# HKUST-Aerial-Robotics/Omni-swarm

Measured on AMD Instinct MI355X. Metric: keyframes/sec (4x fisheye 600x480) + p50 loop-match ms @ 100k-frame DB, higher is better.
Workload: dtype f16

## Files before the change

### omni-swarm_amd/csrc/config.hip

```cpp
#include "config.h"

#include <atomic>
#include <cerrno>
#include <climits>
#include <cstdlib>

namespace omni {

const CfgOption kCfgOptions[CFG_COUNT] = {
    {"OMNI_CONV_V1", 0, 0, 3, CFG_VARIANT, "fp16 3x3 layers: 0 = production (conv1a fused into the ping-pong conv1b, register-stationary cin=128); 1 = generic kernel, 2 = persistent LDS-DMA kernel, "
                                           "3 = ping-pong without the conv1a fusion -- 1-3 exist only in the test build of the library (lib_test/)"},
    {"OMNI_RS_TRN", -1, -1, 1, CFG_VARIANT, "register-stationary kernel of the unpooled cin=128 fp16 layers: tile orientation, -1 = the one with fewer tiles, 0 = plain, 1 = transposed"},
    {"OMNI_DET16", 1, 0, 1, CFG_VARIANT, "detector head of the fp16 and OMNI_PREC_SPLIT paths on v_mfma_f32_32x32x16_f16 with split (hi, lo) operands (0: the exact-f32 MFMA kernel)"},
    {"OMNI_SP_SPARSE_DESC", 1, 0, 1, CFG_VARIANT, "convDb + descriptor norm only at the cells around the key points (0: dense descriptor map)"},
    {"OMNI_SP_SPARSE_DA", 1, 0, 1, CFG_VARIANT, "convDa only at those cells too (fp16 and OMNI_PREC_SPLIT; 0: dense convDa)"},
    {"OMNI_SP_FUSED_CAND", 1, 0, 1, CFG_VARIANT, "getKeyPoints' threshold inside the detector head's epilogue + window masks from the candidate list (0: sp_cand_kernel re-reads the heat map)"},
    {"OMNI_SP_SPLIT_DB", 1, 0, 1, CFG_VARIANT, "OMNI_PREC_SPLIT: convDb + descriptor norm at the key points' cells with split (hi, lo) operands on the fp16 matrix cores (0: exact-f32 MFMA convolution)"},
    {"OMNI_SP_MASK_SKIP", 1, 0, 1, CFG_VARIANT, "fp16: the tiles inside the constant region of the fisheye mask are left out of the tile walk (0: every tile)"},
    {"OMNI_SP_MASK_SKIP_SPLIT", 1, 0, 1, CFG_VARIANT, "the same for OMNI_PREC_SPLIT"},
    {"OMNI_SPLIT_FUSE1A", 1, 0, 1, CFG_VARIANT, "OMNI_PREC_SPLIT: conv1a built inside the conv1b kernel from the u8 image (0: separate exact-f32 conv1a pass)"},
    {"OMNI_SPLIT_WINO", 7, 0, 15, CFG_VARIANT, "OMNI_PREC_SPLIT: the cin = 64 layers as Winograd F(2x2,3x3) kernels with split operands (conv_wino.hip), bit 0 = conv1b (with the conv1a "
                                                "fusion), 1 = conv2a, 2 = conv2b, 3 = conv3a (off by default: same time as the direct kernel, profiles/r06g); 0: the direct kernels of conv_split.hip"},
    {"OMNI_SPLIT_TRN", -1, -1, 1, CFG_VARIANT, "OMNI_PREC_SPLIT cin=128 kernel: tile orientation, as OMNI_RS_TRN"},
    {"OMNI_CONV_XCD", 1, 0, 1, CFG_VARIANT, "persistent convolution kernels derive (cout group, tile walk) from an XCD-aware block id: the cout groups of a pixel tile and its neighbours "
                                           "share one L2 (0: plain blockIdx; process-wide, same results either way)"},
    {"OMNI_SP_PROFILE_MASK", 0, 0, 1, CFG_TUNING, "omni_sp_profile times the stages with the fisheye mask on (what the key-frame pipeline runs)"},
    {"OMNI_PP_U8", 1, 0, 1, CFG_VARIANT, "fp16 conv1a inside conv1b's kernel: matrix-core operands straight from the image bytes (0: through the 256-entry u8 -> (hi, lo) table in LDS)"},
    {"OMNI_PP_TRACE", 0, 0, 1, CFG_DEBUG, "s_memtime trace of the ping-pong conv kernel on stderr"},
    {"OMNI_PP_DBG", 0, 0, 255, CFG_DEBUG, "ping-pong conv kernel timing ablations (WRONG results)"},
    {"OMNI_RS_TRACE", 0, 0, 1, CFG_DEBUG, "s_memtime trace of the register-stationary kernel"},
    {"OMNI_SPLIT_TRACE", 0, 0, 1, CFG_DEBUG, "s_memtime trace of the split-precision kernel"},
    {"OMNI_SPLIT_DBG", 0, 0, 3, CFG_DEBUG, "split-precision kernel timing ablations: 1 = no stores, 2 = every DMA reads tile 0 (WRONG results)"},
    {"OMNI_WINO_TRACE", 0, 0, 1, CFG_DEBUG, "s_memtime trace of the Winograd split kernel"},
    {"OMNI_ROCTX", 0, 0, 1, CFG_DEBUG, "roctx ranges around upload / SuperPoint / MobileNetVLAD / post-processing / BF match / index add + search / exchange and the host loop's "
                                      "stages (rocprofv3 --marker-trace; the library is resolved by dlopen)"},
    {"OMNI_VLAD_BIG", 0, 0, 128, CFG_TUNING, "64 / 128: the 64- / 128-pixel tiles of the unfused block kernel (measured slower at 600x480)"},
    {"OMNI_VLAD_STEM_FUSE", 1, 0, 1, CFG_VARIANT, "stem + block 0 in one kernel (0: two kernels)"},
    {"OMNI_VLAD_UNFUSED", 0, 0, 1, CFG_VARIANT, "1: every block as expand / depthwise / project launches"},
    {"OMNI_VLAD_MFMA", 1, 0, 1, CFG_VARIANT, "late blocks' 1x1 convolutions on the matrix cores"},
    {"OMNI_VLAD_SBLOCK", 1, 0, 1, CFG_VARIANT, "fused split-fp16 block kernel (vlad_s.hip)"},
    {"OMNI_VLAD_MBLOCK_PX", 2048, 0, 1 << 24, CFG_TUNING, "fused matrix-core block kernel for blocks of at most this many input pixels per image (0 disables)"},
    {"OMNI_VLAD_MFMA_PX", 0, 0, 1 << 24, CFG_TUNING, "> 0: matrix-core 1x1 convolutions for blocks of at most this many input pixels per image (default 2048)"},
    {"OMNI_VLAD_FC_MFMA", 1, 0, 1, CFG_VARIANT, "the final FC on the matrix cores (0: VALU kernel)"},
    {"OMNI_VLAD_MBLOCK_CPW", 0, 0, 64, CFG_TUNING, "hidden-layer split of the matrix-core block kernel: chunks per workgroup (0 = no split; measured: does not pay)"},
    {"OMNI_VLAD_SB_LDSPAD", 0, 0, 160 * 1024, CFG_DEBUG, "extra LDS bytes per workgroup of the split block kernel (occupancy A/B)"},
// ... 119 lines not shown
```

### omni-swarm_amd/csrc/conv.h

```cpp
#pragma once
#include "common.h"
#include "tile_walk.h"

namespace omni {

#define CONV_TH 8
#define CONV_TW 32
#define RS_TH 6
#define RS_TW 32
int conv_rs_pool_tile_rows();
#define CONV_COUT_TILE 64
#define CONV_CIN_CHUNK 64

static inline size_t conv_packed_elems(int cin, int cout, int ksize) { return (size_t)cin * cout * ksize * ksize; }

void conv_pack_weights_f16(const float* w_oihw, int cin, int cout, int ksize, __half* out);
void conv_pack_weights_f32(const float* w_oihw, int cin, int cout, int ksize, float* out);

struct ConvArgs {
    const void* in;
    void* out;
    const void* w_packed;
    const float* bias;
    int batch, H, W, cin, cout, ksize;
    int in_cstride = 0;
    bool relu, pool;
    bool out_f32;
    int n_cu = 0;
    const void* zero_page = nullptr;
    float split_inv = 0.f;
    int variant = 0;
    int skip_ty0 = 0, skip_ty1 = 0, skip_tx0 = 0, skip_tx1 = 0;
};
int conv_mfma(hipStream_t stream, int precision, const ConvArgs& a);
int conv_read_pixel_f16(hipStream_t stream, const void* map, int Ho, int Wo, int C, int y, int x, void* vec);
int conv_fill_rect_f16(hipStream_t stream, void* map, int batch, int Ho, int Wo, int C, int y0, int y1, int x0, int x1, const void* vec);
int conv_read_pixel_bytes(hipStream_t stream, const void* map, int64_t row_bytes, int64_t org_bytes, int pix_bytes, int y, int x, void* vec);
int conv_fill_rect_bytes(hipStream_t stream, void* map, int batch, int64_t img_bytes, int64_t row_bytes, int64_t org_bytes, int pix_bytes, int y0, int y1, int x0, int x1,
                         const void* vec);

float conv_pack_weights_split(const float* w_oihw, int cin, int cout, uint16_t* out);
float conv_split_act_scale();
int conv_split(hipStream_t stream, const ConvArgs& a);
int conv1a_split(hipStream_t stream, const uint8_t* gray, int stride, int batch, int H, int W, int fisheye_mask, const float* w, const float* bias,
                 const float* u8_lut, void* out_split, int skip_tr0 = 0, int skip_tr1 = 0);
int split_to_nchw_f32(hipStream_t stream, const void* in_split, float* out, int batch, int C, int H, int W);
void conv1a_split_pack_fused(const float* w , const float* bias , uint16_t* frag );
int conv1ab_split_fused(hipStream_t stream, const ConvArgs& a, const uint8_t* gray, int gstride, int fisheye_mask, const void* w1a_frag, const uint32_t* lut_hl);
float conv_pack_weights_wino(const float* w_oihw, int cin, int cout, uint16_t* out);
// ... 59 lines not shown
```

### omni-swarm_amd/csrc/conv.hip

```cpp
#include "config.h"
#include "conv.h"
#include <type_traits>

namespace omni {

typedef _Float16 half8_t __attribute__((ext_vector_type(8)));
typedef _Float16 half4_t __attribute__((ext_vector_type(4)));
typedef float floatx16 __attribute__((ext_vector_type(16)));
typedef float floatx4 __attribute__((ext_vector_type(4)));

template <typename T, int KG, int EPL>
static void pack_weights(const float* w, int cin, int cout, int ks, T* out) {
    const int taps = ks * ks, n_ct = cout / 64, n_ch = cin / 64;
    size_t o = 0;
    for (int ct = 0; ct < n_ct; ++ct)
        for (int ch = 0; ch < n_ch; ++ch)
            for (int tap = 0; tap < taps; ++tap)
                for (int kg = 0; kg < KG; ++kg)
                    for (int m = 0; m < 2; ++m)
                        for (int l = 0; l < 64; ++l)
                            for (int e = 0; e < EPL; ++e) {
                                const int co = ct * 64 + m * 32 + (l & 31);
                                const int ci = ch * 64 + kg * (64 / KG) + (l >> 5) * EPL + e;
                                const float v = w[((size_t)co * cin + ci) * taps + tap];
// ... 810 lines not shown
static int launch_conv_pp(hipStream_t st, const ConvArgs& a, int n_cu) {
    static const int dbg = config_process()[CFG_PP_DBG];
    switch (dbg >> 2) {
        case 1: return launch_conv_pp_abl<POOL, 1>(st, a, n_cu, dbg & 3);
        case 2: return launch_conv_pp_abl<POOL, 2>(st, a, n_cu, dbg & 3);
        case 3: return launch_conv_pp_abl<POOL, 3>(st, a, n_cu, dbg & 3);
        default: return launch_conv_pp_abl<POOL, 0>(st, a, n_cu, dbg & 3);
    }
}

template <int J, int N, typename F>
__device__ __forceinline__ void spl2_for_each(F&& f) {
    if constexpr (J < N) { f(std::integral_constant<int, J>{}); spl2_for_each<J + 1, N>(f); }
}
#define CSP_KP 8
#define RS_ITH (RS_TH + 2)
#define RS_ITW (RS_TW + 2)
#define RS_PIX (RS_ITH * RS_ITW)
#define RS_CHUNKS (RS_PIX * 16)
#define RS_BUF_BYTES (RS_PIX * 256)
#define RS_SMEM (2 * RS_BUF_BYTES + 512)

template <int L>
__device__ __forceinline__ void rs_read(uint32_t row_base , int n, int hh, half8_t& dst) {
    constexpr int kx = L / 64, r = (L / 8) % 8, kg = L % 8;
    constexpr int pc = r * RS_ITW + kx;
    const uint32_t addr = (row_base + pc * 256 + ((((pc + n) & 15) ^ hh) << 4)) ^ (kg << 5);
    asm volatile("ds_read_b128 %0, %1" : "=v"(dst) : "v"(addr));
}
template <int N>
__device__ __forceinline__ void rs_wait(half8_t& f) { asm volatile("s_waitcnt lgkmcnt(%1)" : "+v"(f) : "i"(N)); }

template <int L, typename IssueFn>
__device__ __forceinline__ void rs_steps(uint32_t row_base, int n, int hh, const half8_t (&wreg)[72], floatx16 (&acc)[RS_TH], half8_t (&fb)[3],
                                         IssueFn& issue_piece) {
    if constexpr (L < 192) {
        constexpr int kx = L / 64, r = (L / 8) % 8, kg = L % 8;
        if constexpr (L + 2 < 192) rs_read<L + 2>(row_base, n, hh, fb[(L + 2) % 3]);
        rs_wait<(L + 2 < 192) ? 2 : (L + 1 < 192 ? 1 : 0)>(fb[L % 3]);
        __builtin_amdgcn_sched_barrier(0);
        if constexpr (r >= 0 && r < RS_TH) acc[r] = __builtin_amdgcn_mfma_f32_32x32x16_f16(wreg[(0 * 3 + kx) * 8 + kg], fb[L % 3], acc[r], 0, 0, 0);
        if constexpr (r - 1 >= 0 && r - 1 < RS_TH) acc[r - 1] = __builtin_amdgcn_mfma_f32_32x32x16_f16(wreg[(1 * 3 + kx) * 8 + kg], fb[L % 3], acc[r - 1], 0, 0, 0);
        if constexpr (r - 2 >= 0 && r - 2 < RS_TH) acc[r - 2] = __builtin_amdgcn_mfma_f32_32x32x16_f16(wreg[(2 * 3 + kx) * 8 + kg], fb[L % 3], acc[r - 2], 0, 0, 0);
        __builtin_amdgcn_sched_barrier(0);
        rs_steps<L + 1>(row_base, n, hh, wreg, acc, fb, issue_piece);
    }
}

__global__ void __launch_bounds__(256, 1)
conv3x3_c128_rs_kernel(const _Float16* __restrict__ in, _Float16* __restrict__ out, const _Float16* __restrict__ wp,
                       const float* __restrict__ bias, int H, int W, int cout, int n_cg, int tiles_x, int tiles_y, int batch, int relu,
                       const char* __restrict__ zero_page ,
                       unsigned long long* trace ,
                       TileWalk wk ) {
    extern __shared__ __attribute__((aligned(16))) char smem_raw[];
    const uint32_t lds0 = (uint32_t)(uintptr_t)(__attribute__((address_space(3))) char*)smem_raw;
    const int tid = threadIdx.x, lane = tid & 63;
    const int wave = __builtin_amdgcn_readfirstlane(tid >> 6);
    const int n = lane & 31, hh = lane >> 5;
    const bool tr = trace != nullptr && blockIdx.x == 0 && tid == 0;
    int tk = 0;
    const int bid = xcd_block_id(wk.xcd);
    const int cg = bid % n_cg, wg = bid / n_cg, nwg = gridDim.x / n_cg;
    const int tiles_per_img = wk.act;
    const int total = batch * tiles_per_img;
    const int g32 = cg * 4 + wave;

    half8_t wreg[72];
    {
        const _Float16* wbase = wp + (int64_t)(g32 >> 1) * 2 * 9 * 4096 + (g32 & 1) * 512 + lane * 8;
#pragma unroll
        for (int s2 = 0; s2 < 72; ++s2) {
            const int tap = s2 >> 3, ch = (s2 >> 2) & 1, kg4 = s2 & 3;
            wreg[s2] = *reinterpret_cast<const half8_t*>(wbase + ((ch * 9 + tap) * 4 + kg4) * 1024);
        }
    }
    float* const bias_lds = reinterpret_cast<float*>(smem_raw + 2 * RS_BUF_BYTES);
    if (tid < 128) bias_lds[tid] = bias[cg * 128 + tid];

    auto tile_origin = [&](int t, int& b, int& ty0, int& tx0) {
        b = t / tiles_per_img;
        int ry, rx;
        tile_walk_rc<false>(wk, tiles_x, t - b * tiles_per_img, ry, rx);
        ty0 = ry * RS_TH; tx0 = rx * RS_TW;
    };
    uint32_t goff[17];
    uint32_t hx[4] = {0, 0, 0, 0};
#pragma unroll
    for (int j = 0; j < 17; ++j) {
        const int idx = (wave * 17 + j) * 64 + lane;
        const int pix = idx >> 4, phys = idx & 15;
        const int iy = pix / RS_ITW, ix = pix - iy * RS_ITW;
        goff[j] = (uint32_t)((iy * W + ix) * 256 + ((phys ^ (pix & 15)) << 4));
        hx[j / 5] |= (uint32_t)ix << (6 * (j % 5));
    }
    const uint32_t in_img_bytes = (uint32_t)H * W * 256u;
    auto issue = [&](int t, int which) {
        int b, ty0, tx0;
        tile_origin(t, b, ty0, tx0);
        const int y0 = ty0 - 1, x0 = tx0 - 1;
        const auto rsrc = __builtin_amdgcn_make_buffer_rsrc(const_cast<_Float16*>(in) + (int64_t)b * H * W * 128, 0, in_img_bytes, 0x00020000);
        const uint32_t sorg = (uint32_t)((y0 * W + x0) * 256);
        char* base = smem_raw + which * RS_BUF_BYTES + wave * 17 * 1024;
#pragma unroll
        for (int j = 0; j < 17; ++j) {
            const uint32_t x = (uint32_t)(x0 + (int)((hx[j / 5] >> (6 * (j % 5))) & 63u));
            const uint32_t voff = x < (uint32_t)W ? goff[j] + sorg : 0x80000000u;
#if __HIP_DEVICE_COMPILE__
            __builtin_amdgcn_raw_ptr_buffer_load_lds(rsrc, (__attribute__((address_space(3))) void*)(base + j * 1024), 16, voff, 0, 0, 0);
#else
            (void)rsrc; (void)base; (void)voff;
#endif
        }
    };
    int t = wg;
    if (t < total) issue(t, 0);
    asm volatile("s_waitcnt vmcnt(0)" ::: "memory");
    __syncthreads();

    int cur = 0;
    for (; t < total; t += nwg, cur ^= 1) {
        const int tn = t + nwg;
        if (tr && tk < 8) { trace[tk * 8 + 0] = __builtin_amdgcn_s_memtime(); trace[tk * 8 + 6] = (unsigned long long)t; }
        if (tn < total) issue(tn, cur ^ 1);
        if (tr && tk < 8) trace[tk * 8 + 1] = __builtin_amdgcn_s_memtime();
        auto issue_piece = [&](int) {};
        const uint32_t row_base = lds0 + cur * RS_BUF_BYTES + n * 256;
        floatx16 acc[RS_TH];
#pragma unroll
        for (int f = 0; f < RS_TH; ++f)
#pragma unroll
            for (int i = 0; i < 16; ++i) acc[f][i] = 0.f;
        half8_t fb[3];
        rs_read<0>(row_base, n, hh, fb[0]);
        rs_read<1>(row_base, n, hh, fb[1]);
        __builtin_amdgcn_sched_barrier(0);
        rs_steps<0>(row_base, n, hh, wreg, acc, fb, issue_piece);
        if (tr && tk < 8) trace[tk * 8 + 2] = __builtin_amdgcn_s_memtime();

        {
            int b, ty0, tx0;
            tile_origin(t, b, ty0, tx0);
            const int ox = tx0 + n;
            float4 bs[4];
#pragma unroll
            for (int g = 0; g < 4; ++g) bs[g] = *reinterpret_cast<const float4*>(bias_lds + wave * 32 + 8 * g + 4 * hh);
#pragma unroll
            for (int f2 = 0; f2 < RS_TH / 2; ++f2) {
                const int oy = ty0 + 2 * f2;
                float v[16];
#pragma unroll
                for (int i = 0; i < 16; ++i) {
                    const float q = vmax_med3(acc[2 * f2][i], acc[2 * f2 + 1][i]);
                    v[i] = vmax_med3(q, dpp_swap_pairs(q));
                }
                _Float16* o = out + (((int64_t)b * (H >> 1) + (oy >> 1)) * (W >> 1) + (ox >> 1)) * cout + g32 * 32;
                store_frag16<false>(v, bs, o, hh, relu, (oy < H) && (ox < W) && !(n & 1));
            }
        }
        if (tr && tk < 8) trace[tk * 8 + 3] = __builtin_amdgcn_s_memtime();
        asm volatile("s_waitcnt vmcnt(0)" ::: "memory");
        if (tr && tk < 8) trace[tk * 8 + 4] = __builtin_amdgcn_s_memtime();
        __syncthreads();
        if (tr && tk < 8) { trace[tk * 8 + 5] = __builtin_amdgcn_s_memtime(); ++tk; }
    }
}

static int launch_conv_rs(hipStream_t st, const ConvArgs& a, int n_cu) {
    auto kfn = conv3x3_c128_rs_kernel;
    OMNI_HIP_TRY(hipFuncSetAttribute((const void*)kfn, hipFuncAttributeMaxDynamicSharedMemorySize, (int)RS_SMEM));
    const int tiles_x = cdiv(a.W, RS_TW), tiles_y = cdiv(a.H, RS_TH), n_cg = a.cout / 128;
    TileWalk wk;
    if (int rc = tile_walk_plan(wk, "conv_rs", tiles_x, tiles_y, a.skip_ty0, a.skip_ty1, a.skip_tx0, a.skip_tx1)) return rc;
    wk.xcd = config_process()[CFG_CONV_XCD];
    const int total = a.batch * wk.act;
    const int per_cg = tile_walk_grid(n_cu, n_cg, total);
    OMNI_REQUIRE(a.zero_page, OMNI_ERR_INVALID, "conv: ConvArgs.zero_page is not set");
    const char* zero_page = reinterpret_cast<const char*>(a.zero_page);
    static const bool want_trace = config_process()[CFG_RS_TRACE] != 0;
    static unsigned long long* trace_dev = nullptr;
    if (want_trace) {
        if (!trace_dev) OMNI_HIP_TRY(hipMalloc((void**)&trace_dev, 64 * 8));
        OMNI_HIP_TRY(hipMemsetAsync(trace_dev, 0, 64 * 8, st));
    }
    hipLaunchKernelGGL(kfn, dim3(per_cg * n_cg), dim3(256), RS_SMEM, st, reinterpret_cast<const _Float16*>(a.in),
                       reinterpret_cast<_Float16*>(a.out), reinterpret_cast<const _Float16*>(a.w_packed), a.bias, a.H, a.W, a.cout, n_cg,
                       tiles_x, tiles_y, a.batch, a.relu ? 1 : 0, zero_page, want_trace ? trace_dev : nullptr, wk);
    OMNI_LAUNCH_CHECK();
    if (want_trace) {
        unsigned long long h[64];
        OMNI_HIP_TRY(hipMemcpyAsync(h, trace_dev, sizeof(h), hipMemcpyDeviceToHost, st));
        OMNI_HIP_TRY(hipStreamSynchronize(st));
        static int launches = 0;
        if (launches++ / 4 == 5)
            for (int k = 0; k < 8; ++k)
                fprintf(stderr, "rs trace H=%d W=%d cout=%d tile %llu (ty %llu tx %llu): issue %llu mfma %llu epilogue %llu wait %llu zerofix+barrier %llu | total %llu\n",
                        a.H, a.W, a.cout, h[k * 8 + 6], (h[k * 8 + 6] % (tiles_x * tiles_y)) / tiles_x, (h[k * 8 + 6] % (tiles_x * tiles_y)) % tiles_x,
                        h[k * 8 + 1] - h[k * 8], h[k * 8 + 2] - h[k * 8 + 1], h[k * 8 + 3] - h[k * 8 + 2], h[k * 8 + 4] - h[k * 8 + 3],
                        h[k * 8 + 5] - h[k * 8 + 4], h[k * 8 + 5] - h[k * 8]);
    }
    return OMNI_OK;
}

#define RS2_RING 3
template <int TH> struct Rs2Cfg {
    static constexpr int ITH = TH + 2, PIX = ITH * RS_ITW, NPIECES = (PIX * 16 + 63) / 64, PPW = (NPIECES + 3) / 4, BUF = NPIECES * 1024, NL = 3 * ITH * 8;
    static constexpr size_t smem() { return 2 * (size_t)BUF + 512; }
};
template <int L, int ITH>
__device__ __forceinline__ void rs2_read(uint32_t row_base , int n, int hh, half8_t& dst) {
    constexpr int kx = L / (ITH * 8), r = (L / 8) % ITH, kg = L % 8;
    constexpr int pc = r * RS_ITW + kx;
    const uint32_t addr = (row_base + pc * 256 + ((((pc + n) & 15) ^ hh) << 4)) ^ (kg << 5);
    asm volatile("ds_read_b128 %0, %1" : "=v"(dst) : "v"(addr));
}
template <int TH> constexpr int rs2_nmfma(int L) { const int r = (L / 8) % (TH + 2); int c = 0; for (int ky = 0; ky < 3; ++ky) if (r - ky >= 0 && r - ky < TH) ++c; return c; }
template <int TH> constexpr int rs2_count_before(int L, int want) { int c = 0; for (int l = 0; l < L; ++l) c += rs2_nmfma<TH>(l) == want ? 1 : 0; return c; }
// ... 206 lines not shown
    static DynSmemState smem_state;
    OMNI_HIP_TRY(ensure_dyn_smem(smem_state, (const void*)kfn, Rs2Cfg<TH>::smem()));
    const int tiles_x = cdiv(a.W, TRN ? TH : RS_TW), tiles_y = cdiv(a.H, TRN ? RS_TW : TH), n_cg = a.cout / 128;
    OMNI_REQUIRE((int64_t)a.H * a.W * 256 < (1ll << 31) && (int64_t)a.H * a.W * a.cout * 2 < (1ll << 31), OMNI_ERR_INVALID, "conv_rs2: image too large for 32-bit offsets");
    TileWalk wk;
    if (int rc = TRN ? tile_walk_plan(wk, "conv_rs2", tiles_x, tiles_y, 0, 0, 0, 0)
                     : tile_walk_plan(wk, "conv_rs2", tiles_x, tiles_y, a.skip_ty0, a.skip_ty1, a.skip_tx0, a.skip_tx1)) return rc;
    wk.xcd = config_process()[CFG_CONV_XCD];
    const int total = a.batch * wk.act;
    const int per_cg = tile_walk_grid(n_cu, n_cg, total);
    hipLaunchKernelGGL(kfn, dim3(per_cg * n_cg), dim3(256), Rs2Cfg<TH>::smem(), st, reinterpret_cast<const _Float16*>(a.in), reinterpret_cast<_Float16*>(a.out),
                       reinterpret_cast<const _Float16*>(a.w_packed), a.bias, a.H, a.W, a.cout, n_cg, tiles_x, tiles_y, a.batch, a.relu ? 1 : 0, wk);
    OMNI_LAUNCH_CHECK();
    return OMNI_OK;
}
int conv_rs_pool_tile_rows() { return RS_TH; }

template <int S, bool TRN>
__device__ __forceinline__ void spc_steps(uint32_t base, const half8_t (&wreg)[72], floatx16& acc, half8_t (&fb)[3]) {
    if constexpr (S < 72) {
        constexpr int o = S / 8, kg = S % 8, tap = TRN ? o : (o % 3) * 3 + o / 3;
        if constexpr (S + 2 < 72) {
            constexpr int o2 = (S + 2) / 8, kg2 = (S + 2) % 8, tap2 = TRN ? o2 : (o2 % 3) * 3 + o2 / 3;
            asm volatile("ds_read_b128 %0, %1 offset:%2" : "=v"(fb[(S + 2) % 3]) : "v"(base), "i"(tap2 * 256 + kg2 * 32));
        }
        asm volatile("s_waitcnt lgkmcnt(%1)" : "+v"(fb[S % 3]) : "i"((S + 2 < 72) ? 2 : (S + 1 < 72 ? 1 : 0)));
        __builtin_amdgcn_sched_barrier(0);
        acc = __builtin_amdgcn_mfma_f32_32x32x16_f16(wreg[tap * 8 + kg], fb[S % 3], acc, 0, 0, 0);
        __builtin_amdgcn_sched_barrier(0);
        spc_steps<S + 1, TRN>(base, wreg, acc, fb);
    }
// ... 221 lines not shown
int conv_mfma(hipStream_t st, int precision, const ConvArgs& a) {
    OMNI_REQUIRE(a.cin % 64 == 0 && a.cout % 64 == 0, OMNI_ERR_INVALID, "conv_mfma: cin=%d cout=%d must be multiples of 64", a.cin, a.cout);
    OMNI_REQUIRE(a.ksize == 1 || a.ksize == 3, OMNI_ERR_INVALID, "conv_mfma: ksize=%d", a.ksize);
    OMNI_REQUIRE(!a.pool || (a.H % 2 == 0 && a.W % 2 == 0), OMNI_ERR_INVALID, "pooling needs even H, W");
    OMNI_REQUIRE(!(a.pool && a.ksize == 1), OMNI_ERR_INVALID, "1x1 + pool not instantiated");
    if (precision == OMNI_PREC_F16 && a.ksize == 3 && a.cin == 64 && !a.out_f32 && (a.in_cstride == 0 || a.in_cstride == 64) && a.n_cu > 0 && a.zero_page &&
        a.variant != 1) {
#ifdef OMNI_TEST_VARIANTS
        if (a.variant == 2) return a.pool ? launch_conv_c64<true>(st, a, a.n_cu) : launch_conv_c64<false>(st, a, a.n_cu);
#endif
        return a.pool ? launch_conv_pp<true>(st, a, a.n_cu) : launch_conv_pp<false>(st, a, a.n_cu);
    }
    if (precision == OMNI_PREC_F16 && a.ksize == 3 && a.cin == 128 && a.cout % 128 == 0 && !a.out_f32 && (a.in_cstride == 0 || a.in_cstride == 128) &&
        a.n_cu > 0 && a.zero_page && a.variant == 0 && (!a.pool || a.H % 2 == 0))
    {
        if (a.pool) return launch_conv_rs(st, a, a.n_cu);
        return rs2_transposed(a.H, a.W) ? launch_conv_rs2<false, true>(st, a, a.n_cu) : launch_conv_rs2<false, false>(st, a, a.n_cu);
    }
    if (precision == OMNI_PREC_F16) {
#ifdef OMNI_TEST_VARIANTS
        if (a.ksize == 3) return a.pool ? launch_conv<_Float16, 3, true>(st, a) : launch_conv<_Float16, 3, false>(st, a);
#else
        OMNI_REQUIRE(a.ksize != 3, OMNI_ERR_INVALID, "conv_mfma: no production fp16 kernel for a 3x3 layer with cin=%d cout=%d in_cstride=%d (the generic one is only built into the test library)",
                     a.cin, a.cout, a.in_cstride);
#endif
        return launch_conv<_Float16, 1, false>(st, a);
    } else {
        if (a.ksize == 3) return a.pool ? launch_conv<float, 3, true>(st, a) : launch_conv<float, 3, false>(st, a);
        return launch_conv<float, 1, false>(st, a);
    }
}
// ... 852 lines not shown
```

### omni-swarm_amd/csrc/superpoint.hip

```cpp
#include <algorithm>
#include <vector>

#include "config.h"
#include "conv.h"
#include "sp_post.h"

namespace {
struct LayerDef { const char* name; int cin, cout, ks; };
const LayerDef kLayers[OMNI_SP_NUM_LAYERS] = {
    {"conv1a", 1, 64, 3},  {"conv1b", 64, 64, 3},   {"conv2a", 64, 64, 3},   {"conv2b", 64, 64, 3},
    {"conv3a", 64, 128, 3}, {"conv3b", 128, 128, 3}, {"conv4a", 128, 128, 3}, {"conv4b", 128, 128, 3},
    {"convPa", 128, 256, 3}, {"convPb", 256, 65, 1}, {"convDa", 128, 256, 3}, {"convDb", 256, 256, 1}};
enum { L1A = 0, L1B, L2A, L2B, L3A, L3B, L4A, L4B, LPA, LPB, LDA, LDB };
enum { ST_CONV1A = 0, ST_CONV1B, ST_CONV2A, ST_CONV2B, ST_CONV3A, ST_CONV3B, ST_CONV4A, ST_CONV4B, ST_HEADS_A,
       ST_DET_TAIL, ST_DESC_TAIL, ST_POST, ST_COUNT };
const char* kStageNames[OMNI_SP_NUM_STAGES] = {
    "conv1a", "conv1b+pool", "conv2a", "conv2b+pool", "conv3a", "conv3b+pool", "conv4a", "conv4b", "convPa|convDa",
    "convPb+softmax+d2s", "convDb+l2norm", "nms+topk+describe", "", "", "", ""};
}

struct omni_sp {
    omni_ctx* ctx = nullptr;
    omni::Config cfg;
    int W = 0, H = 0, Hc = 0, Wc = 0, max_num = 0, max_batch = 0, precision = 0, pca_dim = 0, desc_dim = 256;
// ... 77 lines not shown
    for (auto& k : ks) k = omni_sp::MaskSkip{};
    int a = m0 + 1, b = (m1 == h) ? h - 1 : m1 - 2, c = 0, d = w - 1;
    if (split && b >= a) {
        omni_sp::MaskSkip& k = ks[0];
        k.ty0 = (a + 7) / 8; k.ty1 = (b + 1) / 8; k.tx0 = 0; k.tx1 = (w + 31) / 32;
        if (k.ty1 <= k.ty0) k.ty0 = k.ty1 = k.tx0 = k.tx1 = 0;
        k.oy0 = k.ty0 * 8; k.oy1 = k.ty1 * 8 < h ? k.ty1 * 8 : h; k.ox0 = 0; k.ox1 = k.ty1 > k.ty0 ? w : 0;
        k.oh = h; k.ow = w; k.oc = 64;
        k.frac = (double)(k.ty1 - k.ty0) / ((h + 7) / 8);
    }
    const bool pool[5] = {true, false, true, false, true};
    const int chans[5] = {64, 64, 64, 128, 128};
    static_assert(CONV_TW == 32, "tile width");
    const int TW = 32;
    for (int i = 0; i < 5; ++i) {
        const int TH = split ? (i == 4 ? 2 : 4) : (i == 4 ? conv_rs_pool_tile_rows() : CONV_TH);
        a += 1; b -= 1; c += 1; d -= 1;
        omni_sp::MaskSkip& k = ks[1 + i];
        if (b < a || d < c) break;
        k.ty0 = (a + TH - 1) / TH; k.ty1 = (b + 1) / TH; k.tx0 = (c + TW - 1) / TW; k.tx1 = (d + 1) / TW;
        if (k.ty1 <= k.ty0 || k.tx1 <= k.tx0) k.ty0 = k.ty1 = k.tx0 = k.tx1 = 0;
        k.frac = (double)(k.ty1 - k.ty0) * (k.tx1 - k.tx0) / ((double)((h + TH - 1) / TH) * ((w + TW - 1) / TW));
        const int f = pool[i] ? 2 : 1;
        k.oy0 = k.ty0 * TH / f; k.oy1 = k.ty1 * TH / f; k.ox0 = k.tx0 * TW / f; k.ox1 = k.tx1 * TW / f;
        if (pool[i]) { a = (a + 1) / 2; b = (b - 1) >> 1; c = (c + 1) / 2; d = (d - 1) >> 1; h /= 2; w /= 2; }
        k.oh = h; k.ow = w; k.oc = chans[i];
    }
}

static int sp_plan_mask_skip(omni_sp* s) {
    s->mask_skip = false;
// ... 726 lines not shown
```

Measured before the change: 2739.

## Replace pooled cin=128 fp16 conv3b kernel with new 16x16 MFMA c128 kernel

Swaps the register-stationary pooled cin=128 kernel, which used 32x32x16 MFMA, 256 threads, 6-row tiles and 72 weight registers, for a new kernel in conv_c128.hip. The new kernel uses 16-wide cout groups with 36 weight registers per lane, 512 threads, 4-row tiles and a 3-deep LDS read ring. The epilogue does fused ReLU and pack with buffer stores, and waits on a partial vmcnt so stores can overlap the next tile. The aim is more waves per CU and lower register pressure. The cost is smaller tiles, so more halo reloads and tile overhead, and the mask-skip plan is remapped between 6-row and 4-row tiles.

```diff
diff --git a/omni-swarm_amd/csrc/config.hip b/omni-swarm_amd/csrc/config.hip
--- a/omni-swarm_amd/csrc/config.hip
+++ b/omni-swarm_amd/csrc/config.hip
@@ -8,9 +8,9 @@
 namespace omni {
 
 const CfgOption kCfgOptions[CFG_COUNT] = {
-    {"OMNI_CONV_V1", 0, 0, 3, CFG_VARIANT, "fp16 3x3 layers: 0 = production (conv1a fused into the ping-pong conv1b, register-stationary cin=128); 1 = generic kernel, 2 = persistent LDS-DMA kernel, "
+    {"OMNI_CONV_V1", 0, 0, 3, CFG_VARIANT, "fp16 3x3 layers: 0 = production (conv1a fused into the ping-pong conv1b, cin=128 layers on conv_c128.hip (pooled) and v5); 1 = generic kernel, 2 = persistent LDS-DMA kernel, "
                                            "3 = ping-pong without the conv1a fusion -- 1-3 exist only in the test build of the library (lib_test/)"},
-    {"OMNI_RS_TRN", -1, -1, 1, CFG_VARIANT, "register-stationary kernel of the unpooled cin=128 fp16 layers: tile orientation, -1 = the one with fewer tiles, 0 = plain, 1 = transposed"},
+    {"OMNI_RS_TRN", -1, -1, 1, CFG_VARIANT, "register-stationary kernel (v5) of the unpooled cin=128 fp16 layers: tile orientation, -1 = the one with fewer tiles, 0 = plain, 1 = transposed"},
     {"OMNI_DET16", 1, 0, 1, CFG_VARIANT, "detector head of the fp16 and OMNI_PREC_SPLIT paths on v_mfma_f32_32x32x16_f16 with split (hi, lo) operands (0: the exact-f32 MFMA kernel)"},
     {"OMNI_SP_SPARSE_DESC", 1, 0, 1, CFG_VARIANT, "convDb + descriptor norm only at the cells around the key points (0: dense descriptor map)"},
     {"OMNI_SP_SPARSE_DA", 1, 0, 1, CFG_VARIANT, "convDa only at those cells too (fp16 and OMNI_PREC_SPLIT; 0: dense convDa)"},
@@ -28,7 +28,7 @@
     {"OMNI_PP_U8", 1, 0, 1, CFG_VARIANT, "fp16 conv1a inside conv1b's kernel: matrix-core operands straight from the image bytes (0: through the 256-entry u8 -> (hi, lo) table in LDS)"},
     {"OMNI_PP_TRACE", 0, 0, 1, CFG_DEBUG, "s_memtime trace of the ping-pong conv kernel on stderr"},
     {"OMNI_PP_DBG", 0, 0, 255, CFG_DEBUG, "ping-pong conv kernel timing ablations (WRONG results)"},
-    {"OMNI_RS_TRACE", 0, 0, 1, CFG_DEBUG, "s_memtime trace of the register-stationary kernel"},
+    {"OMNI_RS_TRACE", 0, 0, 1, CFG_DEBUG, "s_memtime trace of the pooled fp16 cin=128 kernel (conv_c128.hip)"},
     {"OMNI_SPLIT_TRACE", 0, 0, 1, CFG_DEBUG, "s_memtime trace of the split-precision kernel"},
     {"OMNI_SPLIT_DBG", 0, 0, 3, CFG_DEBUG, "split-precision kernel timing ablations: 1 = no stores, 2 = every DMA reads tile 0 (WRONG results)"},
     {"OMNI_WINO_TRACE", 0, 0, 1, CFG_DEBUG, "s_memtime trace of the Winograd split kernel"},
diff --git a/omni-swarm_amd/csrc/conv.h b/omni-swarm_amd/csrc/conv.h
--- a/omni-swarm_amd/csrc/conv.h
+++ b/omni-swarm_amd/csrc/conv.h
@@ -6,9 +6,9 @@
 
 #define CONV_TH 8
 #define CONV_TW 32
-#define RS_TH 6
 #define RS_TW 32
-int conv_rs_pool_tile_rows();
+#define C128_TW 32
+int conv_c128_pool_tile_rows();
 #define CONV_COUT_TILE 64
 #define CONV_CIN_CHUNK 64
 
@@ -33,6 +33,7 @@
     int skip_ty0 = 0, skip_ty1 = 0, skip_tx0 = 0, skip_tx1 = 0;
 };
 int conv_mfma(hipStream_t stream, int precision, const ConvArgs& a);
+int conv_c128(hipStream_t stream, const ConvArgs& a);
 int conv_read_pixel_f16(hipStream_t stream, const void* map, int Ho, int Wo, int C, int y, int x, void* vec);
 int conv_fill_rect_f16(hipStream_t stream, void* map, int batch, int Ho, int Wo, int C, int y0, int y1, int x0, int x1, const void* vec);
 int conv_read_pixel_bytes(hipStream_t stream, const void* map, int64_t row_bytes, int64_t org_bytes, int pix_bytes, int y, int x, void* vec);
diff --git a/omni-swarm_amd/csrc/conv.hip b/omni-swarm_amd/csrc/conv.hip
--- a/omni-swarm_amd/csrc/conv.hip
+++ b/omni-swarm_amd/csrc/conv.hip
@@ -848,193 +848,7 @@
     if constexpr (J < N) { f(std::integral_constant<int, J>{}); spl2_for_each<J + 1, N>(f); }
 }
 #define CSP_KP 8
-#define RS_ITH (RS_TH + 2)
 #define RS_ITW (RS_TW + 2)
-#define RS_PIX (RS_ITH * RS_ITW)
-#define RS_CHUNKS (RS_PIX * 16)
-#define RS_BUF_BYTES (RS_PIX * 256)
-#define RS_SMEM (2 * RS_BUF_BYTES + 512)
-
-template <int L>
-__device__ __forceinline__ void rs_read(uint32_t row_base , int n, int hh, half8_t& dst) {
-    constexpr int kx = L / 64, r = (L / 8) % 8, kg = L % 8;
-    constexpr int pc = r * RS_ITW + kx;
-    const uint32_t addr = (row_base + pc * 256 + ((((pc + n) & 15) ^ hh) << 4)) ^ (kg << 5);
-    asm volatile("ds_read_b128 %0, %1" : "=v"(dst) : "v"(addr));
-}
-template <int N>
-__device__ __forceinline__ void rs_wait(half8_t& f) { asm volatile("s_waitcnt lgkmcnt(%1)" : "+v"(f) : "i"(N)); }
-
-template <int L, typename IssueFn>
-__device__ __forceinline__ void rs_steps(uint32_t row_base, int n, int hh, const half8_t (&wreg)[72], floatx16 (&acc)[RS_TH], half8_t (&fb)[3],
-                                         IssueFn& issue_piece) {
-    if constexpr (L < 192) {
-        constexpr int kx = L / 64, r = (L / 8) % 8, kg = L % 8;
-        if constexpr (L + 2 < 192) rs_read<L + 2>(row_base, n, hh, fb[(L + 2) % 3]);
-        rs_wait<(L + 2 < 192) ? 2 : (L + 1 < 192 ? 1 : 0)>(fb[L % 3]);
-        __builtin_amdgcn_sched_barrier(0);
-        if constexpr (r >= 0 && r < RS_TH) acc[r] = __builtin_amdgcn_mfma_f32_32x32x16_f16(wreg[(0 * 3 + kx) * 8 + kg], fb[L % 3], acc[r], 0, 0, 0);
-        if constexpr (r - 1 >= 0 && r - 1 < RS_TH) acc[r - 1] = __builtin_amdgcn_mfma_f32_32x32x16_f16(wreg[(1 * 3 + kx) * 8 + kg], fb[L % 3], acc[r - 1], 0, 0, 0);
-        if constexpr (r - 2 >= 0 && r - 2 < RS_TH) acc[r - 2] = __builtin_amdgcn_mfma_f32_32x32x16_f16(wreg[(2 * 3 + kx) * 8 + kg], fb[L % 3], acc[r - 2], 0, 0, 0);
-        __builtin_amdgcn_sched_barrier(0);
-        rs_steps<L + 1>(row_base, n, hh, wreg, acc, fb, issue_piece);
-    }
-}
-
-__global__ void __launch_bounds__(256, 1)
-conv3x3_c128_rs_kernel(const _Float16* __restrict__ in, _Float16* __restrict__ out, const _Float16* __restrict__ wp,
-                       const float* __restrict__ bias, int H, int W, int cout, int n_cg, int tiles_x, int tiles_y, int batch, int relu,
-                       const char* __restrict__ zero_page ,
-                       unsigned long long* trace ,
-                       TileWalk wk ) {
-    extern __shared__ __attribute__((aligned(16))) char smem_raw[];
-    const uint32_t lds0 = (uint32_t)(uintptr_t)(__attribute__((address_space(3))) char*)smem_raw;
-    const int tid = threadIdx.x, lane = tid & 63;
-    const int wave = __builtin_amdgcn_readfirstlane(tid >> 6);
-    const int n = lane & 31, hh = lane >> 5;
-    const bool tr = trace != nullptr && blockIdx.x == 0 && tid == 0;
-    int tk = 0;
-    const int bid = xcd_block_id(wk.xcd);
-    const int cg = bid % n_cg, wg = bid / n_cg, nwg = gridDim.x / n_cg;
-    const int tiles_per_img = wk.act;
-    const int total = batch * tiles_per_img;
-    const int g32 = cg * 4 + wave;
-
-    half8_t wreg[72];
-    {
-        const _Float16* wbase = wp + (int64_t)(g32 >> 1) * 2 * 9 * 4096 + (g32 & 1) * 512 + lane * 8;
-#pragma unroll
-        for (int s2 = 0; s2 < 72; ++s2) {
-            const int tap = s2 >> 3, ch = (s2 >> 2) & 1, kg4 = s2 & 3;
-            wreg[s2] = *reinterpret_cast<const half8_t*>(wbase + ((ch * 9 + tap) * 4 + kg4) * 1024);
-        }
-    }
-    float* const bias_lds = reinterpret_cast<float*>(smem_raw + 2 * RS_BUF_BYTES);
-    if (tid < 128) bias_lds[tid] = bias[cg * 128 + tid];
-
-    auto tile_origin = [&](int t, int& b, int& ty0, int& tx0) {
-        b = t / tiles_per_img;
-        int ry, rx;
-        tile_walk_rc<false>(wk, tiles_x, t - b * tiles_per_img, ry, rx);
-        ty0 = ry * RS_TH; tx0 = rx * RS_TW;
-    };
-    uint32_t goff[17];
-    uint32_t hx[4] = {0, 0, 0, 0};
-#pragma unroll
-    for (int j = 0; j < 17; ++j) {
-        const int idx = (wave * 17 + j) * 64 + lane;
-        const int pix = idx >> 4, phys = idx & 15;
-        const int iy = pix / RS_ITW, ix = pix - iy * RS_ITW;
-        goff[j] = (uint32_t)((iy * W + ix) * 256 + ((phys ^ (pix & 15)) << 4));
-        hx[j / 5] |= (uint32_t)ix << (6 * (j % 5));
-    }
-    const uint32_t in_img_bytes = (uint32_t)H * W * 256u;
-    auto issue = [&](int t, int which) {
-        int b, ty0, tx0;
-        tile_origin(t, b, ty0, tx0);
-        const int y0 = ty0 - 1, x0 = tx0 - 1;
-        const auto rsrc = __builtin_amdgcn_make_buffer_rsrc(const_cast<_Float16*>(in) + (int64_t)b * H * W * 128, 0, in_img_bytes, 0x00020000);
-        const uint32_t sorg = (uint32_t)((y0 * W + x0) * 256);
-        char* base = smem_raw + which * RS_BUF_BYTES + wave * 17 * 1024;
-#pragma unroll
-        for (int j = 0; j < 17; ++j) {
-            const uint32_t x = (uint32_t)(x0 + (int)((hx[j / 5] >> (6 * (j % 5))) & 63u));
-            const uint32_t voff = x < (uint32_t)W ? goff[j] + sorg : 0x80000000u;
-#if __HIP_DEVICE_COMPILE__
-            __builtin_amdgcn_raw_ptr_buffer_load_lds(rsrc, (__attribute__((address_space(3))) void*)(base + j * 1024), 16, voff, 0, 0, 0);
-#else
-            (void)rsrc; (void)base; (void)voff;
-#endif
-        }
-    };
-    int t = wg;
-    if (t < total) issue(t, 0);
-    asm volatile("s_waitcnt vmcnt(0)" ::: "memory");
-    __syncthreads();
-
-    int cur = 0;
-    for (; t < total; t += nwg, cur ^= 1) {
-        const int tn = t + nwg;
-        if (tr && tk < 8) { trace[tk * 8 + 0] = __builtin_amdgcn_s_memtime(); trace[tk * 8 + 6] = (unsigned long long)t; }
-        if (tn < total) issue(tn, cur ^ 1);
-        if (tr && tk < 8) trace[tk * 8 + 1] = __builtin_amdgcn_s_memtime();
-        auto issue_piece = [&](int) {};
-        const uint32_t row_base = lds0 + cur * RS_BUF_BYTES + n * 256;
-        floatx16 acc[RS_TH];
-#pragma unroll
-        for (int f = 0; f < RS_TH; ++f)
-#pragma unroll
-            for (int i = 0; i < 16; ++i) acc[f][i] = 0.f;
-        half8_t fb[3];
-        rs_read<0>(row_base, n, hh, fb[0]);
-        rs_read<1>(row_base, n, hh, fb[1]);
-        __builtin_amdgcn_sched_barrier(0);
-        rs_steps<0>(row_base, n, hh, wreg, acc, fb, issue_piece);
-        if (tr && tk < 8) trace[tk * 8 + 2] = __builtin_amdgcn_s_memtime();
-
-        {
-            int b, ty0, tx0;
-            tile_origin(t, b, ty0, tx0);
-            const int ox = tx0 + n;
-            float4 bs[4];
-#pragma unroll
-            for (int g = 0; g < 4; ++g) bs[g] = *reinterpret_cast<const float4*>(bias_lds + wave * 32 + 8 * g + 4 * hh);
-#pragma unroll
-            for (int f2 = 0; f2 < RS_TH / 2; ++f2) {
-                const int oy = ty0 + 2 * f2;
-                float v[16];
-#pragma unroll
-                for (int i = 0; i < 16; ++i) {
-                    const float q = vmax_med3(acc[2 * f2][i], acc[2 * f2 + 1][i]);
-                    v[i] = vmax_med3(q, dpp_swap_pairs(q));
-                }
-                _Float16* o = out + (((int64_t)b * (H >> 1) + (oy >> 1)) * (W >> 1) + (ox >> 1)) * cout + g32 * 32;
-                store_frag16<false>(v, bs, o, hh, relu, (oy < H) && (ox < W) && !(n & 1));
-            }
-        }
-        if (tr && tk < 8) trace[tk * 8 + 3] = __builtin_amdgcn_s_memtime();
-        asm volatile("s_waitcnt vmcnt(0)" ::: "memory");
-        if (tr && tk < 8) trace[tk * 8 + 4] = __builtin_amdgcn_s_memtime();
-        __syncthreads();
-        if (tr && tk < 8) { trace[tk * 8 + 5] = __builtin_amdgcn_s_memtime(); ++tk; }
-    }
-}
-
-static int launch_conv_rs(hipStream_t st, const ConvArgs& a, int n_cu) {
-    auto kfn = conv3x3_c128_rs_kernel;
-    OMNI_HIP_TRY(hipFuncSetAttribute((const void*)kfn, hipFuncAttributeMaxDynamicSharedMemorySize, (int)RS_SMEM));
-    const int tiles_x = cdiv(a.W, RS_TW), tiles_y = cdiv(a.H, RS_TH), n_cg = a.cout / 128;
-    TileWalk wk;
-    if (int rc = tile_walk_plan(wk, "conv_rs", tiles_x, tiles_y, a.skip_ty0, a.skip_ty1, a.skip_tx0, a.skip_tx1)) return rc;
-    wk.xcd = config_process()[CFG_CONV_XCD];
-    const int total = a.batch * wk.act;
-    const int per_cg = tile_walk_grid(n_cu, n_cg, total);
-    OMNI_REQUIRE(a.zero_page, OMNI_ERR_INVALID, "conv: ConvArgs.zero_page is not set");
-    const char* zero_page = reinterpret_cast<const char*>(a.zero_page);
-    static const bool want_trace = config_process()[CFG_RS_TRACE] != 0;
-    static unsigned long long* trace_dev = nullptr;
-    if (want_trace) {
-        if (!trace_dev) OMNI_HIP_TRY(hipMalloc((void**)&trace_dev, 64 * 8));
-        OMNI_HIP_TRY(hipMemsetAsync(trace_dev, 0, 64 * 8, st));
-    }
-    hipLaunchKernelGGL(kfn, dim3(per_cg * n_cg), dim3(256), RS_SMEM, st, reinterpret_cast<const _Float16*>(a.in),
-                       reinterpret_cast<_Float16*>(a.out), reinterpret_cast<const _Float16*>(a.w_packed), a.bias, a.H, a.W, a.cout, n_cg,
-                       tiles_x, tiles_y, a.batch, a.relu ? 1 : 0, zero_page, want_trace ? trace_dev : nullptr, wk);
-    OMNI_LAUNCH_CHECK();
-    if (want_trace) {
-        unsigned long long h[64];
-        OMNI_HIP_TRY(hipMemcpyAsync(h, trace_dev, sizeof(h), hipMemcpyDeviceToHost, st));
-        OMNI_HIP_TRY(hipStreamSynchronize(st));
-        static int launches = 0;
-        if (launches++ / 4 == 5)
-            for (int k = 0; k < 8; ++k)
-                fprintf(stderr, "rs trace H=%d W=%d cout=%d tile %llu (ty %llu tx %llu): issue %llu mfma %llu epilogue %llu wait %llu zerofix+barrier %llu | total %llu\n",
-                        a.H, a.W, a.cout, h[k * 8 + 6], (h[k * 8 + 6] % (tiles_x * tiles_y)) / tiles_x, (h[k * 8 + 6] % (tiles_x * tiles_y)) % tiles_x,
-                        h[k * 8 + 1] - h[k * 8], h[k * 8 + 2] - h[k * 8 + 1], h[k * 8 + 3] - h[k * 8 + 2], h[k * 8 + 4] - h[k * 8 + 3],
-                        h[k * 8 + 5] - h[k * 8 + 4], h[k * 8 + 5] - h[k * 8]);
-    }
-    return OMNI_OK;
-}
 
 #define RS2_RING 3
 template <int TH> struct Rs2Cfg {
@@ -1271,7 +1085,6 @@
     OMNI_LAUNCH_CHECK();
     return OMNI_OK;
 }
-int conv_rs_pool_tile_rows() { return RS_TH; }
 
 template <int S, bool TRN>
 __device__ __forceinline__ void spc_steps(uint32_t base, const half8_t (&wreg)[72], floatx16& acc, half8_t (&fb)[3]) {
@@ -1523,7 +1336,7 @@
     if (precision == OMNI_PREC_F16 && a.ksize == 3 && a.cin == 128 && a.cout % 128 == 0 && !a.out_f32 && (a.in_cstride == 0 || a.in_cstride == 128) &&
         a.n_cu > 0 && a.zero_page && a.variant == 0 && (!a.pool || a.H % 2 == 0))
     {
-        if (a.pool) return launch_conv_rs(st, a, a.n_cu);
+        if (a.pool) return conv_c128(st, a);
         return rs2_transposed(a.H, a.W) ? launch_conv_rs2<false, true>(st, a, a.n_cu) : launch_conv_rs2<false, false>(st, a, a.n_cu);
     }
     if (precision == OMNI_PREC_F16) {
diff --git a/omni-swarm_amd/csrc/conv_c128.hip b/omni-swarm_amd/csrc/conv_c128.hip
--- /dev/null
+++ b/omni-swarm_amd/csrc/conv_c128.hip
@@ -0,0 +1,259 @@
+#include "config.h"
+#include "conv.h"
+#include <type_traits>
+
+namespace omni {
+
+typedef _Float16 half8_t __attribute__((ext_vector_type(8)));
+typedef float floatx4 __attribute__((ext_vector_type(4)));
+typedef float float2_t __attribute__((ext_vector_type(2)));
+typedef _Float16 half2_t __attribute__((ext_vector_type(2)));
+typedef uint32_t u2_t __attribute__((ext_vector_type(2)));
+
+#define C128_ITW (C128_TW + 2)
+#define C128_RING 3
+#define C128_TH_POOL 4
+#define C128_SKIP_TH 6
+
+namespace {
+
+template <int J, int N, typename F>
+__device__ __forceinline__ void c128_for_each(F&& f) {
+    if constexpr (J < N) { f(std::integral_constant<int, J>{}); c128_for_each<J + 1, N>(f); }
+}
+__device__ __forceinline__ float c128_max(float a, float b) { return __builtin_amdgcn_fmed3f(a, b, __builtin_inff()); }
+__device__ __forceinline__ float c128_swap_pairs(float v) {
+    return __builtin_bit_cast(float, __builtin_amdgcn_update_dpp(0, __builtin_bit_cast(int, v), 0xB1, 0xF, 0xF, false));
+}
+__device__ __forceinline__ uint32_t c128_pack_relu(float a, float b) {
+    const int ia = __builtin_bit_cast(int, a), ib = __builtin_bit_cast(int, b);
+    float2_t f; f[0] = __builtin_bit_cast(float, ia > 0 ? ia : 0); f[1] = __builtin_bit_cast(float, ib > 0 ? ib : 0);
+    return __builtin_bit_cast(uint32_t, __builtin_convertvector(f, half2_t));
+}
+
+}
+
+__host__ __device__ constexpr int c128_tap(int o) { return (o % 3) * 3 + o / 3; }
+
+__device__ __forceinline__ void c128_load_weights(const _Float16* __restrict__ wp, int g16, int lane, half8_t (&wreg)[36]) {
+    const int co = g16 * 16 + (lane & 15), q = lane >> 4;
+    const _Float16* wb = wp + (int64_t)(co >> 6) * 2 * 9 * 4096 + ((co >> 5) & 1) * 512 + ((co & 31) + 32 * (q & 1)) * 8;
+#pragma unroll
+    for (int s = 0; s < 36; ++s) {
+        const int o = s >> 2, c = s & 3, tap = c128_tap(o), ch = c >> 1, kg = (c & 1) * 2 + (q >> 1);
+        wreg[s] = *reinterpret_cast<const half8_t*>(wb + ((ch * 9 + tap) * 4 + kg) * 1024);
+    }
+}
+
+int conv_c128_pool_tile_rows() { return C128_SKIP_TH; }
+
+template <int TH> struct C128Cfg {
+    static constexpr int ITH = TH + 2, PIX = ITH * C128_ITW, NPIECES = (PIX * 16 + 63) / 64, PPW = (NPIECES + 7) / 8, BUF = NPIECES * 1024;
+    static constexpr int NP = 2 * ITH + 1;
+    static constexpr size_t smem() { return 2 * (size_t)BUF; }
+    static_assert(2 * ITH <= 15, "swizzle phase beyond 15");
+};
+
+template <int L, int ITH>
+__device__ __forceinline__ void c128_read(const uint32_t (&ab)[2 * ITH + 1], half8_t& dst) {
+    constexpr int kx = L / (ITH * 8), r = (L / 8) % ITH, c = (L / 2) % 4, hf = L % 2;
+    constexpr int pc = r * C128_ITW + kx + 16 * hf;
+    const uint32_t a = c ? (ab[2 * r + kx] ^ (uint32_t)(c << 6)) : ab[2 * r + kx];
+    asm volatile("ds_read_b128 %0, %1 offset:%2" : "=v"(dst) : "v"(a), "i"(pc * 256));
+}
+template <int L, int TH>
+__device__ __forceinline__ void c128_steps(const uint32_t (&ab)[2 * TH + 5], const half8_t (&wreg)[36], floatx4 (&acc)[TH][2], half8_t (&fb)[C128_RING]) {
+    constexpr int ITH = TH + 2, NL = 3 * ITH * 8, D = C128_RING - 1;
+    if constexpr (L < NL) {
+        constexpr int kx = L / (ITH * 8), r = (L / 8) % ITH, c = (L / 2) % 4, hf = L % 2;
+        if constexpr (L + D < NL) c128_read<L + D, ITH>(ab, fb[(L + D) % C128_RING]);
+        asm volatile("s_waitcnt lgkmcnt(%1)" : "+v"(fb[L % C128_RING]) : "i"((L + D < NL) ? D : (NL - 1 - L)));
+        __builtin_amdgcn_sched_barrier(0);
+        if constexpr (r < TH) acc[r][hf] = __builtin_amdgcn_mfma_f32_16x16x32_f16(wreg[(kx * 3 + 0) * 4 + c], fb[L % C128_RING], acc[r][hf], 0, 0, 0);
+        if constexpr (r - 1 >= 0 && r - 1 < TH) acc[r - 1][hf] = __builtin_amdgcn_mfma_f32_16x16x32_f16(wreg[(kx * 3 + 1) * 4 + c], fb[L % C128_RING], acc[r - 1][hf], 0, 0, 0);
+        if constexpr (r - 2 >= 0 && r - 2 < TH) acc[r - 2][hf] = __builtin_amdgcn_mfma_f32_16x16x32_f16(wreg[(kx * 3 + 2) * 4 + c], fb[L % C128_RING], acc[r - 2][hf], 0, 0, 0);
+        __builtin_amdgcn_sched_barrier(0);
+        c128_steps<L + 1, TH>(ab, wreg, acc, fb);
+    }
+}
+
+template <int TH>
+__global__ void __launch_bounds__(512, 1)
+conv3x3_c128_pool_kernel(const _Float16* __restrict__ in, _Float16* __restrict__ out, const _Float16* __restrict__ wp, const float* __restrict__ bias,
+                    int H, int W, int cout, int n_cg, int tiles_x, int batch,
+                    unsigned long long* trace ,
+                    TileWalk wk ) {
+    using C = C128Cfg<TH>;
+    constexpr int ITH = C::ITH, PPW = C::PPW, NPIECES = C::NPIECES, NP = C::NP;
+    static_assert(TH % 2 == 0, "pooled tiles: even rows");
+    constexpr int NST = TH;
+    extern __shared__ __attribute__((aligned(16))) char smem_raw[];
+    const uint32_t lds0 = (uint32_t)(uintptr_t)(__attribute__((address_space(3))) char*)smem_raw;
+    const int tid = threadIdx.x, lane = tid & 63;
+    const int wave = __builtin_amdgcn_readfirstlane(tid >> 6);
+    const int j = lane & 15, q = lane >> 4;
+    const int bid = xcd_block_id(wk.xcd);
+    const int cg = bid % n_cg, wg = bid / n_cg, nwg = gridDim.x / n_cg;
+    const int tiles_per_img = wk.act;
+    const int total = batch * tiles_per_img;
+    const int g16 = cg * 8 + wave;
+    const bool tr = trace != nullptr && blockIdx.x == 0 && tid == 0;
+    int tk = 0;
+
+    half8_t wreg[36];
+    c128_load_weights(wp, g16, lane, wreg);
+    const float4 bs = *reinterpret_cast<const float4*>(bias + g16 * 16 + 4 * q);
+
+    auto tile_origin = [&](int t, int& b, int& ty0, int& tx0) {
+        b = t / tiles_per_img;
+        int ry, rx;
+        tile_walk_rc<false>(wk, tiles_x, t - b * tiles_per_img, ry, rx);
+        ty0 = ry * TH; tx0 = rx * C128_TW;
+    };
+    uint32_t goff[PPW];
+    uint32_t hx[(PPW + 4) / 5];
+#pragma unroll
+    for (int i = 0; i < (PPW + 4) / 5; ++i) hx[i] = 0;
+#pragma unroll
+    for (int jj = 0; jj < PPW; ++jj) {
+        int piece = wave * PPW + jj;
+        piece = piece < NPIECES ? piece : NPIECES - 1;
+        const int idx = piece * 64 + lane;
+        const int pix = idx >> 4, phys = idx & 15;
+        const int iy = pix / C128_ITW, ix = pix - iy * C128_ITW;
+        goff[jj] = (uint32_t)((iy * W + ix) * 256 + ((phys ^ (pix & 15)) << 4));
+        hx[jj / 5] |= (uint32_t)(ix & 63) << (6 * (jj % 5));
+    }
+    const uint32_t in_img_bytes = (uint32_t)H * W * 256u;
+    struct Src { __amdgpu_buffer_rsrc_t r; uint32_t sorg; int x0; };
+    auto source = [&](int t) -> Src {
+        int b, ty0, tx0;
+        tile_origin(t, b, ty0, tx0);
+        Src s;
+        s.r = __builtin_amdgcn_make_buffer_rsrc(const_cast<_Float16*>(in) + (int64_t)b * H * W * 128, 0, in_img_bytes, 0x00020000);
+        s.x0 = tx0 - 1;
+        s.sorg = (uint32_t)(((ty0 - 1) * W + s.x0) * 256);
+        return s;
+    };
+    auto dma_piece = [&](const Src& s, int which, auto JC) {
+        constexpr int jj = decltype(JC)::value;
+        int piece = wave * PPW + jj;
+        piece = piece < NPIECES ? piece : NPIECES - 1;
+        const uint32_t x = (uint32_t)(s.x0 + (int)((hx[jj / 5] >> (6 * (jj % 5))) & 63u));
+        const uint32_t voff = x < (uint32_t)W ? goff[jj] + s.sorg : 0x80000000u;
+#if __HIP_DEVICE_COMPILE__
+        __builtin_amdgcn_raw_ptr_buffer_load_lds(s.r, (__attribute__((address_space(3))) void*)(smem_raw + which * C::BUF + piece * 1024), 16, voff, 0, 0, 0);
+#else
+        (void)s; (void)which; (void)piece; (void)voff;
+#endif
+    };
+    int t = wg;
+    if (t < total) {
+        const Src s0 = source(t);
+        c128_for_each<0, PPW>([&](auto JC) { dma_piece(s0, 0, JC); });
+    }
+    asm volatile("s_waitcnt vmcnt(0)" ::: "memory");
+    __syncthreads();
+
+    const uint32_t out_img_bytes = (uint32_t)((int64_t)(H >> 1) * (W >> 1) * cout * 2);
+    int cur = 0;
+    for (; t < total; t += nwg, cur ^= 1) {
+        const int tn = t + nwg;
+        if (tr && tk < 8) { trace[tk * 8 + 0] = __builtin_amdgcn_s_memtime(); trace[tk * 8 + 6] = (unsigned long long)t; }
+        if (tn < total) {
+            const Src sn = source(tn);
+            c128_for_each<0, PPW>([&](auto JC) { dma_piece(sn, cur ^ 1, JC); });
+        }
+        if (tr && tk < 8) trace[tk * 8 + 1] = __builtin_amdgcn_s_memtime();
+        __builtin_amdgcn_sched_barrier(0);
+        uint32_t ab[NP];
+        const uint32_t buf = lds0 + cur * C::BUF + j * 256;
+#pragma unroll
+        for (int P = 0; P < NP; ++P) ab[P] = buf + ((((j + P) & 15) ^ q) << 4);
+        floatx4 acc[TH][2];
+#pragma unroll
+        for (int f = 0; f < TH; ++f)
+#pragma unroll
+            for (int h = 0; h < 2; ++h) acc[f][h] = floatx4{0.f, 0.f, 0.f, 0.f};
+        half8_t fb[C128_RING];
+        c128_for_each<0, C128_RING - 1>([&](auto LC) { c128_read<decltype(LC)::value, ITH>(ab, fb[decltype(LC)::value]); });
+        __builtin_amdgcn_sched_barrier(0);
+        c128_steps<0, TH>(ab, wreg, acc, fb);
+        if (tr && tk < 8) trace[tk * 8 + 2] = __builtin_amdgcn_s_memtime();
+
+        {
+            int b, ty0, tx0;
+            tile_origin(t, b, ty0, tx0);
+            const __amdgpu_buffer_rsrc_t oimg = __builtin_amdgcn_make_buffer_rsrc(out + (int64_t)b * (out_img_bytes / 2), 0, out_img_bytes, 0x00020000);
+#pragma unroll
+            for (int f2 = 0; f2 < TH / 2; ++f2)
+#pragma unroll
+                for (int h = 0; h < 2; ++h) {
+                    float v[4];
+#pragma unroll
+                    for (int i = 0; i < 4; ++i) {
+                        const float m = c128_max(acc[2 * f2][h][i], acc[2 * f2 + 1][h][i]);
+                        v[i] = c128_max(m, c128_swap_pairs(m));
+                    }
+                    const int oy = ty0 + 2 * f2, ox = tx0 + 16 * h + j;
+                    const uint32_t off = (oy < H && ox < W && !(j & 1)) ? (uint32_t)((((oy >> 1) * (W >> 1) + (ox >> 1)) * cout + g16 * 16 + 4 * q) * 2) : 0x80000000u;
+                    const u2_t d = {c128_pack_relu(v[0] + bs.x, v[1] + bs.y), c128_pack_relu(v[2] + bs.z, v[3] + bs.w)};
+                    __builtin_amdgcn_raw_buffer_store_b64(d, oimg, off, 0, 0);
+                }
+        }
+        if (tr && tk < 8) trace[tk * 8 + 3] = __builtin_amdgcn_s_memtime();
+        asm volatile("s_waitcnt vmcnt(%0)" :: "i"(NST) : "memory");
+        if (tr && tk < 8) trace[tk * 8 + 4] = __builtin_amdgcn_s_memtime();
+        __builtin_amdgcn_sched_barrier(0);
+        __builtin_amdgcn_s_barrier();
+        __builtin_amdgcn_sched_barrier(0);
+        if (tr && tk < 8) { trace[tk * 8 + 5] = __builtin_amdgcn_s_memtime(); ++tk; }
+    }
+}
+
+template <int TH>
+static int launch_conv_c128(hipStream_t st, const ConvArgs& a) {
+    using C = C128Cfg<TH>;
+    auto kfn = conv3x3_c128_pool_kernel<TH>;
+    static DynSmemState smem_state;
+    OMNI_HIP_TRY(ensure_dyn_smem(smem_state, (const void*)kfn, C::smem()));
+    const int tiles_x = cdiv(a.W, C128_TW), tiles_y = cdiv(a.H, TH), n_cg = a.cout / 128;
+    OMNI_REQUIRE((int64_t)a.H * a.W * 256 < (1ll << 31) && (int64_t)a.H * a.W * a.cout * 2 < (1ll << 31), OMNI_ERR_INVALID, "conv_c128: image too large for 32-bit offsets");
+    int sy0 = cdiv(a.skip_ty0 * C128_SKIP_TH, TH), sy1 = a.skip_ty1 * C128_SKIP_TH / TH;
+    if (sy1 <= sy0) sy0 = sy1 = 0;
+    TileWalk wk;
+    if (int rc = tile_walk_plan(wk, "conv_c128", tiles_x, tiles_y, sy0, sy1, a.skip_tx0, a.skip_tx1)) return rc;
+    wk.xcd = config_process()[CFG_CONV_XCD];
+    const int total = a.batch * wk.act;
+    const int per_cg = tile_walk_grid(a.n_cu, n_cg, total);
+    static const bool want_trace = config_process()[CFG_RS_TRACE] != 0;
+    static unsigned long long* trace_dev = nullptr;
+    if (want_trace) {
+        if (!trace_dev) OMNI_HIP_TRY(hipMalloc((void**)&trace_dev, 64 * 8));
+        OMNI_HIP_TRY(hipMemsetAsync(trace_dev, 0, 64 * 8, st));
+    }
+    hipLaunchKernelGGL(kfn, dim3(per_cg * n_cg), dim3(512), C::smem(), st, reinterpret_cast<const _Float16*>(a.in), reinterpret_cast<_Float16*>(a.out),
+                       reinterpret_cast<const _Float16*>(a.w_packed), a.bias, a.H, a.W, a.cout, n_cg, tiles_x, a.batch, want_trace ? trace_dev : nullptr, wk);
+    OMNI_LAUNCH_CHECK();
+    if (want_trace) {
+        unsigned long long h[64];
+        OMNI_HIP_TRY(hipMemcpyAsync(h, trace_dev, sizeof(h), hipMemcpyDeviceToHost, st));
+        OMNI_HIP_TRY(hipStreamSynchronize(st));
+        static int launches = 0;
+        if (launches++ == 5)
+            for (int k = 0; k < 8; ++k)
+                fprintf(stderr, "c128 trace H=%d W=%d cout=%d tile %llu: issue %llu mfma %llu epilogue %llu wait %llu barrier %llu | total %llu\n",
+                        a.H, a.W, a.cout, h[k * 8 + 6], h[k * 8 + 1] - h[k * 8], h[k * 8 + 2] - h[k * 8 + 1], h[k * 8 + 3] - h[k * 8 + 2],
+                        h[k * 8 + 4] - h[k * 8 + 3], h[k * 8 + 5] - h[k * 8 + 4], h[k * 8 + 5] - h[k * 8]);
+    }
+    return OMNI_OK;
+}
+
+int conv_c128(hipStream_t st, const ConvArgs& a) {
+    OMNI_REQUIRE(a.relu && a.pool, OMNI_ERR_INVALID, "conv_c128: instantiated with ReLU + 2 x 2 max-pool in its epilogue (conv3b)");
+    OMNI_REQUIRE(a.cin == 128 && a.cout % 128 == 0 && a.ksize == 3 && a.H % 2 == 0 && a.W % 2 == 0, OMNI_ERR_INVALID, "conv_c128: cin=%d cout=%d H=%d W=%d",
+                 a.cin, a.cout, a.H, a.W);
+    return launch_conv_c128<C128_TH_POOL>(st, a);
+}
+
+}
diff --git a/omni-swarm_amd/csrc/superpoint.hip b/omni-swarm_amd/csrc/superpoint.hip
--- a/omni-swarm_amd/csrc/superpoint.hip
+++ b/omni-swarm_amd/csrc/superpoint.hip
@@ -115,7 +115,7 @@
     static_assert(CONV_TW == 32, "tile width");
     const int TW = 32;
     for (int i = 0; i < 5; ++i) {
-        const int TH = split ? (i == 4 ? 2 : 4) : (i == 4 ? conv_rs_pool_tile_rows() : CONV_TH);
+        const int TH = split ? (i == 4 ? 2 : 4) : (i == 4 ? conv_c128_pool_tile_rows() : CONV_TH);
         a += 1; b -= 1; c += 1; d -= 1;
         omni_sp::MaskSkip& k = ks[1 + i];
         if (b < a || d < c) break;
```

Result: no change. 2732, median of 4 (-0.3%).
